# Bojian-Wei/Non-IID-Distributed-Learning-with-Optimal-Mixture-Weights

Measured on AMD Instinct MI355X. Metric: client-rounds/sec (whole node), higher is better.
Workload: dtype f32; 1 GPU; config 2: fedavg, 100 clients x 512 rows, RFF D=2048, C=10, E=2, B=32, 10000 test rows, round=1880, parallel clients; algo=fedavg, clients_total=100, clients_per_gpu=100, rows_per_client=512, D=2048, C=10, epochs=2, batch=32, test_rows=10000, parallelism=clients1

## Files before the change

non-iid-distributed-learning-with-optimal-mixture-weights_amd/_lib.py:

```python
import ctypes as C
import os

import torch

from . import LIB_PATH

_c_f32p = C.POINTER(C.c_float)
_SIGS = {
    'fs_abi_version': (C.c_int, []),
    'fs_last_error': (C.c_char_p, []),
    'fs_tuning_size': (C.c_int64, []),
    'fs_set_tuning': (C.c_int, [C.c_void_p]),
    'fs_set_thread_tuning': (C.c_int, [C.c_void_p]),
    'fs_get_tuning': (C.c_int, [C.c_void_p]),
    'fs_get_process_tuning': (C.c_int, [C.c_void_p]),
    'fs_get_thread_tuning': (C.c_int, [C.c_void_p]),
    'fs_randperm_batch': (C.c_int, [C.c_void_p, C.c_void_p, C.c_void_p, C.c_int64, C.c_void_p, C.c_int]),
    'fs_libsvm_scan': (C.c_int, [C.c_char_p, C.c_void_p, C.c_void_p, C.c_void_p]),
    'fs_libsvm_read': (C.c_int, [C.c_char_p, C.c_int64, C.c_int64, C.c_int, C.c_void_p, C.c_void_p, C.c_int]),
    'fs_randperm_device': (C.c_int, [C.c_void_p, C.c_void_p, C.c_void_p, C.c_int64, C.c_int64, C.c_void_p,
                                     C.c_void_p, C.c_void_p]),
    'fs_local_train_plan': (C.c_int, [C.c_int, C.c_int, C.c_int, C.c_int, C.c_int64, C.c_int64, C.c_int,
                                      C.c_int, C.c_void_p, C.c_void_p]),
    'fs_local_train': (C.c_int, [C.c_void_p, C.c_int64, C.c_void_p, C.c_void_p, C.c_void_p, C.c_void_p,
# ... 49 lines not shown
    'fs_plan_shuffle': (C.c_int, [C.c_void_p, C.c_void_p, C.c_int]),
    'fs_plan_round': (C.c_int, [C.c_void_p, C.c_int, C.c_float, C.c_int, C.c_void_p, C.c_void_p]),
    'fs_plan_eval_flush': (C.c_int, [C.c_void_p, C.c_void_p]),
    'fs_local_train_last_kernel': (C.c_int, []),
    'fs_plan_set_shuffle_chunk': (C.c_int, [C.c_void_p, C.c_int]),
    'fs_plan_shuffle_flush': (C.c_int, [C.c_void_p]),
    'fs_plan_eval_blocks': (C.c_int, [C.c_void_p]),
    'fs_timer_create': (C.c_int, [C.c_void_p]),
    'fs_timer_record': (C.c_int, [C.c_void_p, C.c_void_p]),
    'fs_timer_elapsed_ms': (C.c_int, [C.c_void_p, C.c_void_p, C.c_void_p]),
    'fs_timer_destroy': (C.c_int, [C.c_void_p]),
}

EXPORTS = tuple(_SIGS)
ABI_VERSION = 20

PHASE_TRAIN, PHASE_AGGREGATE, PHASE_EVAL, PHASE_EVAL_DEFER = 1, 2, 4, 8
G_PAIR = 256
G_TEAMS = 512
LT_KERNELS = {1: 'single', 2: 'split', 3: 'dbuf', 4: 'pair', 5: 'pipe', 6: 'teams', 7: 'mb'}
G_PIPE = 1024
ERR_BLOCK = 256
SOLVER_NAMES = {0: 'none', 1: 'reg', 2: 'mc', 3: 'staged', 4: 'global', 5: 'reg2', 6: 'wave', 8: 'quad', 9: 'qmc', 10: 'bin'}
SOLVERS = {v: k for k, v in SOLVER_NAMES.items() if k}


class Tuning(C.Structure):
    _fields_ = [('mix_solver', C.c_int), ('mix_prefetch', C.c_int), ('mix_prefetch_lead', C.c_int),
                ('mix_exact_softmax', C.c_int), ('no_eval_fuse', C.c_int), ('spin_limit', C.c_uint),
                ('inject_timeout', C.c_int), ('train_form', C.c_int),
                ('split_early', C.c_int), ('mix_qmc_lane_clients', C.c_int),
                ('mix_quad_loaders', C.c_int), ('split_teams', C.c_int),
                ('mix_poll_delay', C.c_int), ('split_poll_delay', C.c_int), ('split_pipe', C.c_int),
                ('split_dbuf', C.c_int),
                ('split_mb', C.c_int)]


class PlanDesc(C.Structure):
    _fields_ = [
        ('d_phi', C.c_void_p), ('ld', C.c_int64), ('d_row_off', C.c_void_p), ('d_labels', C.c_void_p),
        ('d_order', C.c_void_p), ('h_n', C.c_void_p),
        ('N', C.c_int), ('C', C.c_int), ('B', C.c_int), ('E', C.c_int), ('G', C.c_int),
        ('d_ws', C.c_void_p), ('ws_bytes', C.c_int64),
        ('chained', C.c_int), ('prox', C.c_int), ('reg', C.c_int), ('mu', C.c_float), ('lam', C.c_float),
        ('d_W_g', C.c_void_p), ('d_W_out', C.c_void_p), ('d_loss_hist', C.c_void_p),
        ('d_p', C.c_void_p), ('d_agg_ws', C.c_void_p), ('agg_ws_floats', C.c_int64), ('agg_chunks', C.c_int),
        ('d_phi_t', C.c_void_p), ('d_labels_t', C.c_void_p), ('n_t', C.c_int), ('d_eval_ws', C.c_void_p),
        ('d_eval_hist', C.c_void_p), ('shuffle_device', C.c_int), ('host_threads', C.c_int),
        ('shuffle_after_train', C.c_int),
        ('loss', C.c_int), ('d_y', C.c_void_p), ('d_y_t', C.c_void_p),
    ]

_lib = None


class FedsimError(RuntimeError):
    pass


def lib():
    global _lib
    if _lib is None:
        path = os.environ.get('FEDSIM_LIB') or LIB_PATH
        if not os.path.exists(path):
            raise FedsimError(
                'libfedsim.so not found at %s -- build it with `python -c "import __graft_entry__ as g; g.build()"` '
                'or `make -C <pkg>/csrc`; there is no CPU fallback' % path)
        h = C.CDLL(path, mode=C.RTLD_GLOBAL)
        for name, (res, args) in _SIGS.items():
            f = getattr(h, name)
            f.restype = res
            f.argtypes = args
        if h.fs_abi_version() != ABI_VERSION:
            raise FedsimError('libfedsim.so ABI %d != %d' % (h.fs_abi_version(), ABI_VERSION))
        if h.fs_tuning_size() != C.sizeof(Tuning):
            raise FedsimError('fs_tuning layout mismatch (%d != %d bytes)' % (h.fs_tuning_size(), C.sizeof(Tuning)))
        if h.fs_plan_desc_size() != C.sizeof(PlanDesc):
            raise FedsimError('fs_plan_desc layout mismatch (%d != %d bytes)' % (h.fs_plan_desc_size(),
                                                                                  C.sizeof(PlanDesc)))
        _lib = h
    return _lib


def get_tuning():
    t = Tuning()
    check(lib().fs_get_tuning(C.byref(t)), 'fs_get_tuning')
    return {k: getattr(t, k) for k, _ in Tuning._fields_}


def last_mix_layout():
    k, nk = C.c_int(0), C.c_int(0)
    check(lib().fs_mix_solve_last_layout(C.byref(k), C.byref(nk)), 'fs_mix_solve_last_layout')
    return k.value, nk.value


class MixPlan(C.Structure):
    _fields_ = [('solver', C.c_int), ('workgroups', C.c_int), ('lane_clients', C.c_int), ('helpers', C.c_int),
                ('lead', C.c_int), ('poll_delay', C.c_int), ('ws_bytes', C.c_int64)]


def mix_plan(N, C_, n_val, epochs, Bv, blocks=1):
    out = MixPlan()
    check(lib().fs_mix_solve_plan(int(N), int(C_), int(n_val), int(epochs), int(Bv), int(blocks), C.byref(out)),
          'fs_mix_solve_plan')
    return {k: getattr(out, k) for k, _ in MixPlan._fields_}


def get_process_tuning():
    t = Tuning()
    check(lib().fs_get_process_tuning(C.byref(t)), 'fs_get_process_tuning')
    return {k: getattr(t, k) for k, _ in Tuning._fields_}


def get_thread_tuning():
    t = Tuning()
    has = lib().fs_get_thread_tuning(C.byref(t))
    if has < 0:
        check(has, 'fs_get_thread_tuning')
    return {k: getattr(t, k) for k, _ in Tuning._fields_} if has else None


def _merged(base, fields):
    cur = dict(base)
    for k, v in fields.items():
        if k not in cur:
            raise KeyError('fs_tuning has no field %r' % k)
        if k == 'mix_solver' and isinstance(v, str):
            v = 0 if v == 'auto' else SOLVERS[v]
        cur[k] = int(v)
    return cur


def set_tuning(**fields):
    prev = get_process_tuning()
    check(lib().fs_set_tuning(C.byref(Tuning(**_merged(prev, fields)))), 'fs_set_tuning')
    return prev


def set_thread_tuning(fields=None):
    if fields is None:
        check(lib().fs_set_thread_tuning(None), 'fs_set_thread_tuning')
        return
    cur = _merged({k: 0 for k, _ in Tuning._fields_}, fields)
    check(lib().fs_set_thread_tuning(C.byref(Tuning(**cur))), 'fs_set_thread_tuning')


class tuning:

    def __init__(self, **fields):
        self.fields = fields

    def __enter__(self):
        own = get_thread_tuning()
        self.thread_prev = own
        if own is not None:
            set_thread_tuning(_merged(own, self.fields))
        else:
            self.prev = set_tuning(**self.fields)
        return self

    def __exit__(self, *exc):
        if self.thread_prev is not None:
            set_thread_tuning(self.thread_prev)
        else:
            check(lib().fs_set_tuning(C.byref(Tuning(**self.prev))), 'fs_set_tuning')
        return False
# ... 85 lines not shown
```

non-iid-distributed-learning-with-optimal-mixture-weights_amd/csrc/randperm.hip:

```cpp
#include "common.h"

namespace fs {

constexpr int MT_N = 624, MT_M = 397;
constexpr int RP_THREADS = 64;

__device__ __forceinline__ uint32_t mt_mix(uint32_t a, uint32_t b, uint32_t c) {
  const uint32_t y = (a & 0x80000000u) | (b & 0x7fffffffu);
  return c ^ (y >> 1) ^ ((y & 1u) ? 0x9908b0dfu : 0u);
}

__device__ __forceinline__ uint32_t mt_temper(uint32_t y) {
  y ^= y >> 11;
  y ^= (y << 7) & 0x9d2c5680u;
  y ^= (y << 15) & 0xefc60000u;
  y ^= y >> 18;
  return y;
}

__device__ void mt_twist(uint32_t* mt) {
  const int lane = threadIdx.x;
  uint32_t v[4];
#pragma unroll
  for (int k = 0; k < 4; ++k) {
    const int i = lane + 64 * k;
    if (i < MT_N - MT_M) v[k] = mt_mix(mt[i], mt[i + 1], mt[i + MT_M]);
  }
  __syncthreads();
#pragma unroll
  for (int k = 0; k < 4; ++k) {
    const int i = lane + 64 * k;
    if (i < MT_N - MT_M) mt[i] = v[k];
  }
  __syncthreads();
#pragma unroll
  for (int k = 0; k < 4; ++k) {
    const int i = (MT_N - MT_M) + lane + 64 * k;
    if (i < 2 * (MT_N - MT_M)) v[k] = mt_mix(mt[i], mt[i + 1], mt[i + MT_M - MT_N]);
  }
  __syncthreads();
#pragma unroll
  for (int k = 0; k < 4; ++k) {
    const int i = (MT_N - MT_M) + lane + 64 * k;
    if (i < 2 * (MT_N - MT_M)) mt[i] = v[k];
  }
  __syncthreads();
#pragma unroll
  for (int k = 0; k < 3; ++k) {
    const int i = 2 * (MT_N - MT_M) + lane + 64 * k;
    if (i < MT_N - 1) v[k] = mt_mix(mt[i], mt[i + 1], mt[i + MT_M - MT_N]);
  }
  __syncthreads();
#pragma unroll
  for (int k = 0; k < 3; ++k) {
    const int i = 2 * (MT_N - MT_M) + lane + 64 * k;
    if (i < MT_N - 1) mt[i] = v[k];
  }
  __syncthreads();
  if (lane == 0) mt[MT_N - 1] = mt_mix(mt[MT_N - 1], mt[0], mt[MT_M - 1]);
  __syncthreads();
}

__device__ __forceinline__ void rp_contract_broken(int32_t* dst, int n, int lane, int stride, uint32_t* err) {
  for (int i = lane; i < n; i += stride) dst[i] = i;
  if (err && lane == 0) __hip_atomic_store(err, 1u, __ATOMIC_RELAXED, __HIP_MEMORY_SCOPE_AGENT);
}

template <bool IN_LDS>
__global__ __launch_bounds__(RP_THREADS) void randperm_kernel(const int64_t* __restrict__ seeds,
                                                             const int64_t* __restrict__ ns,
                                                             const int64_t* __restrict__ offs,
                                                             int32_t* __restrict__ out, int64_t max_n,
                                                             uint32_t* err) {
  extern __shared__ __attribute__((aligned(16))) uint32_t smem_rp[];
  uint32_t* mt = smem_rp;
  uint32_t* rnd = mt + MT_N;
  const int lane = threadIdx.x;
  const int pass = blockIdx.x;
  const int64_t n64 = ns[pass];
  int32_t* dst = out + offs[pass];
  if (n64 > max_n) {
    rp_contract_broken(dst, (int)n64, lane, RP_THREADS, err);
    return;
  }
  const int n = (int)n64;
  int32_t* perm = IN_LDS ? reinterpret_cast<int32_t*>(rnd + MT_N) : dst;
  for (int i = lane; i < n; i += RP_THREADS) perm[i] = i;
  if (lane == 0) {
    uint32_t x = (uint32_t)(uint64_t)seeds[pass];
    mt[0] = x;
    for (int i = 1; i < MT_N; ++i) {
      x = 1812433253u * (x ^ (x >> 30)) + (uint32_t)i;
      mt[i] = x;
    }
  }
  __syncthreads();
  for (int i0 = 0; i0 < n - 1; i0 += MT_N) {
    mt_twist(mt);
    for (int k = lane; k < MT_N; k += RP_THREADS) rnd[k] = mt_temper(mt[k]);
    __syncthreads();
    if (lane == 0) {
      const int i1 = min(n - 1, i0 + MT_N);
      for (int i = i0; i < i1; ++i) {
        const uint32_t z = rnd[i - i0] % (uint32_t)(n - i);
        const int32_t a = perm[i];
        perm[i] = perm[i + z];
        perm[i + z] = a;
      }
    }
    __syncthreads();
  }
  if (IN_LDS)
    for (int i = lane; i < n; i += RP_THREADS) dst[i] = perm[i];
}

constexpr int RL_MAXN = 64;

__global__ __launch_bounds__(64) void randperm_lanes_kernel(const int64_t* __restrict__ seeds,
                                                           const int64_t* __restrict__ ns,
                                                           const int64_t* __restrict__ offs, int64_t npasses,
                                                           int32_t* __restrict__ out, int max_n, uint32_t* err) {
  __shared__ int32_t perm_s[64][RL_MAXN + 1];
  const int lane = threadIdx.x;
  const int64_t pass = (int64_t)blockIdx.x * 64 + lane;
  const bool live = pass < npasses;
  const int n_req = live ? (int)ns[pass] : 0;
  const int n = n_req <= max_n ? n_req : 0;
  if (n_req > max_n && err) __hip_atomic_store(err, 1u, __ATOMIC_RELAXED, __HIP_MEMORY_SCOPE_AGENT);
  int32_t* perm = perm_s[lane];
  uint32_t lo[RL_MAXN], hi[RL_MAXN - 1];
  {
    uint32_t x = live ? (uint32_t)(uint64_t)seeds[pass] : 0u;
    lo[0] = x;
#pragma unroll
    for (int i = 1; i <= MT_M + RL_MAXN - 2; ++i) {
      x = 1812433253u * (x ^ (x >> 30)) + (uint32_t)i;
      if (i < RL_MAXN) lo[i] = x;
      if (i >= MT_M) hi[i - MT_M] = x;
    }
  }
#pragma unroll
  for (int i = 0; i < RL_MAXN; ++i)
    if (i < n) perm[i] = i;
#pragma unroll
  for (int i = 0; i < RL_MAXN - 1; ++i) {
    if (i < n - 1) {
      const uint32_t r = mt_temper(mt_mix(lo[i], lo[i + 1], hi[i]));
      const int z = (int)(r % (uint32_t)(n - i));
      const int32_t a = perm[i];
      perm[i] = perm[i + z];
      perm[i + z] = a;
    }
  }
  if (live) {
    int32_t* dst = out + offs[pass];
    for (int i = 0; i < n; ++i) dst[i] = perm[i];
    for (int i = n; i < n_req; ++i) dst[i] = i;
  }
}

}

using namespace fs;

extern "C" int fs_randperm_device(const int64_t* d_seeds, const int64_t* d_n, const int64_t* d_off, int64_t npasses,
                                  int64_t max_n, int32_t* d_out, uint32_t* d_err, void* stream) {
  FS_REQUIRE(npasses >= 0 && max_n >= 0 && max_n < ((int64_t)1 << 31), "bad sizes");
  if (npasses == 0) return FS_OK;
  FS_REQUIRE(d_seeds && d_n && d_off && d_out, "null pointer");
  hipStream_t st = reinterpret_cast<hipStream_t>(stream);
  if (max_n <= RL_MAXN) {
    hipLaunchKernelGGL(randperm_lanes_kernel, dim3((unsigned)((npasses + 63) / 64)), dim3(64), 0, st, d_seeds, d_n,
                       d_off, npasses, d_out, (int)max_n, d_err);
    FS_LAUNCH_CHECK();
    return FS_OK;
  }
  const size_t lds_small = sizeof(uint32_t) * 2 * MT_N;
  const size_t lds_full = lds_small + sizeof(int32_t) * (size_t)max_n;
  if (lds_full <= 160 * 1024) {
    if (lds_full > 64 * 1024) {
      hipError_t e = hipFuncSetAttribute(reinterpret_cast<const void*>(&randperm_kernel<true>),
                                         hipFuncAttributeMaxDynamicSharedMemorySize, (int)lds_full);
      if (e != hipSuccess) return fail(FS_EHIP, std::string("fs_randperm_device: ") + hipGetErrorString(e));
    }
    hipLaunchKernelGGL(randperm_kernel<true>, dim3((unsigned)npasses), dim3(RP_THREADS), lds_full, st, d_seeds, d_n,
                       d_off, d_out, max_n, d_err);
  } else {
    hipLaunchKernelGGL(randperm_kernel<false>, dim3((unsigned)npasses), dim3(RP_THREADS), lds_small, st, d_seeds, d_n,
                       d_off, d_out, max_n, d_err);
  }
  FS_LAUNCH_CHECK();
  return FS_OK;
}
```

non-iid-distributed-learning-with-optimal-mixture-weights_amd/csrc/round.hip:

```cpp
#include <hip/hip_runtime.h>

#include <algorithm>
#include <atomic>
#include <condition_variable>
#include <cstring>
#include <functional>
#include <mutex>
#include <deque>
#include <thread>
#include <vector>

#include <chrono>
#include <cstdio>

#include "common.h"
#include "finalize.h"
#include "mse_rows.h"
#include "mt_replay.h"

namespace fs {

class Pool {
 public:
  explicit Pool(int nthreads) {
    for (int t = 1; t < nthreads; ++t) th_.emplace_back([this] { loop(); });
  }
  ~Pool() {
    {
      std::lock_guard<std::mutex> lk(m_);
      stop_ = true;
      ++gen_;
    }
    cv_.notify_all();
    for (auto& t : th_) t.join();
  }
  void run(int64_t n, const std::function<void(int64_t)>& fn) {
    if (th_.empty() || n <= 1) {
      for (int64_t i = 0; i < n; ++i) fn(i);
      return;
    }
    {
      std::lock_guard<std::mutex> lk(m_);
      fn_ = &fn;
      n_ = n;
      next_.store(0);
      busy_ = (int)th_.size();
      ++gen_;
    }
    cv_.notify_all();
    work();
    std::unique_lock<std::mutex> lk(m_);
    done_.wait(lk, [this] { return busy_ == 0; });
    fn_ = nullptr;
  }

 private:
  void work() {
    for (;;) {
      const int64_t i = next_.fetch_add(1);
      if (i >= n_) return;
      (*fn_)(i);
    }
  }
  void loop() {
    uint64_t seen = 0;
    for (;;) {
      {
        std::unique_lock<std::mutex> lk(m_);
        cv_.wait(lk, [&] { return gen_ != seen; });
        seen = gen_;
        if (stop_) return;
      }
      work();
      std::lock_guard<std::mutex> lk(m_);
      if (--busy_ == 0) done_.notify_all();
    }
  }
  std::vector<std::thread> th_;
  std::mutex m_;
  std::condition_variable cv_, done_;
  const std::function<void(int64_t)>* fn_ = nullptr;
  int64_t n_ = 0;
  std::atomic<int64_t> next_{0};
  int busy_ = 0;
  uint64_t gen_ = 0;
  bool stop_ = false;
};

}

struct fs_plan {
  fs_plan_desc d;
  std::vector<int64_t> n, off;
  int64_t perm_len = 0;
  int32_t* h_perm[2] = {nullptr, nullptr};
  int32_t* d_perm[2] = {nullptr, nullptr};
  static constexpr int SEED_SLOTS = 4;
  int64_t* h_seed[SEED_SLOTS] = {};
  int64_t* d_seed[SEED_SLOTS] = {};
  int64_t* h_seed_dev[SEED_SLOTS] = {};
  hipEvent_t seed_read[SEED_SLOTS] = {};
  bool seed_pending[SEED_SLOTS] = {};
  bool seed_copy = false;
  int64_t* d_pass = nullptr;
  int64_t max_n = 0;
  int64_t max_client_steps = 0;
  int fuse_E = 0;
  int eval_pending = -1;
  int fin_pending = -1;
  hipStream_t copy = nullptr;
  hipEvent_t uploaded[2] = {nullptr, nullptr};
  hipEvent_t consumed[2] = {nullptr, nullptr};
  bool up_pending[2] = {false, false};
  bool cons_recorded[2] = {false, false};
  int slot_round[2] = {-1, -1};
  int chunk = 1;
  int64_t* d_pass_chunk = nullptr;
  int slot_chunk[2] = {-1, -1};
  int slot_nrounds[2] = {0, 0};
  int slot_waited[2] = {-1, -1};
  int fill_chunk = -1, fill_rounds = 0;
  int job_status = FS_OK;
  std::string job_error;
  fs::Pool* pool = nullptr;
  std::thread coord;
  std::mutex m;
  std::condition_variable cv, done;
  std::deque<std::pair<int, std::vector<int64_t>>> jobs;
  bool stop = false;
};

using namespace fs;

static int hip_fail(const char* what, hipError_t e) {
  return fail(FS_EHIP, std::string(what) + ": " + hipGetErrorString(e));
}

#define FS_HIP(call, what)                          \
  do {                                              \
    hipError_t e_ = (call);                         \
    if (e_ != hipSuccess) return hip_fail(what, e_); \
  } while (0)

extern "C" int64_t fs_plan_desc_size(void) { return (int64_t)sizeof(fs_plan_desc); }

static int run_shuffle_job(fs_plan* p, const int64_t* h_seeds, int t);

static void coordinator(fs_plan* p) {
  for (;;) {
    std::pair<int, std::vector<int64_t>> job;
    {
      std::unique_lock<std::mutex> lk(p->m);
      p->cv.wait(lk, [p] { return p->stop || !p->jobs.empty(); });
      if (p->jobs.empty()) return;
      job = std::move(p->jobs.front());
    }
    const int rc = run_shuffle_job(p, job.second.data(), job.first);
    std::lock_guard<std::mutex> lk(p->m);
    p->jobs.pop_front();
    if (rc != FS_OK && p->job_status == FS_OK) {
      p->job_status = rc;
      p->job_error = fs_last_error();
    }
    p->done.notify_all();
  }
}

extern "C" int fs_plan_destroy(fs_plan* p) {
  if (!p) return FS_OK;
  if (p->coord.joinable()) {
    {
      std::lock_guard<std::mutex> lk(p->m);
      p->stop = true;
    }
    p->cv.notify_all();
    p->coord.join();
  }
  if (p->copy) (void)hipStreamSynchronize(p->copy);
  for (int s = 0; s < 2; ++s) {
    if (p->h_perm[s]) (void)hipHostFree(p->h_perm[s]);
    if (p->d_perm[s]) (void)hipFree(p->d_perm[s]);
    if (p->uploaded[s]) (void)hipEventDestroy(p->uploaded[s]);
    if (p->consumed[s]) (void)hipEventDestroy(p->consumed[s]);
  }
  for (int s = 0; s < fs_plan::SEED_SLOTS; ++s) {
    if (p->h_seed[s]) (void)hipHostFree(p->h_seed[s]);
    if (p->d_seed[s]) (void)hipFree(p->d_seed[s]);
    if (p->seed_read[s]) (void)hipEventDestroy(p->seed_read[s]);
  }
  if (p->d_pass) (void)hipFree(p->d_pass);
  if (p->d_pass_chunk) (void)hipFree(p->d_pass_chunk);
  if (p->copy) (void)hipStreamDestroy(p->copy);
  delete p->pool;
  delete p;
  return FS_OK;
}

extern "C" int fs_plan_create(const fs_plan_desc* desc, fs_plan** out) {
  FS_REQUIRE(desc && out, "null pointer");
  const fs_plan_desc& d = *desc;
  FS_REQUIRE(d.N >= 1 && d.E >= 0 && d.C >= 1 && d.ld >= 64 && d.ld % 64 == 0, "bad sizes");
  FS_REQUIRE(d.loss == 0 || d.loss == 1, "loss must be 0 (cross-entropy) or 1 (MSE)");
  FS_REQUIRE(d.h_n && d.d_phi && d.d_row_off && (d.loss ? (const void*)d.d_y : (const void*)d.d_labels) && d.d_W_g &&
                 d.d_W_out && d.d_loss_hist,
             "null pointer");
  FS_REQUIRE(d.loss == 0 || (d.C == 1 && d.G == 1), "the MSE plan needs C == 1 and G == 1");
  *out = nullptr;
  fs_plan* p = new fs_plan();
  p->d = d;
  int64_t rows = 0;
  for (int j = 0; j < d.N; ++j) {
    if (d.h_n[j] < 0) {
      delete p;
      return fail(FS_EINVAL, "fs_plan_create: negative client size");
    }
    for (int e = 0; e < d.E; ++e) {
      p->n.push_back(d.h_n[j]);
      p->off.push_back((int64_t)d.E * rows + (int64_t)e * d.h_n[j]);
    }
    rows += d.h_n[j];
  }
  p->perm_len = std::max<int64_t>(1, (int64_t)d.E * rows);
  const int64_t P = (int64_t)p->n.size();
  for (int64_t v : p->n) p->max_n = std::max(p->max_n, v);
  {
    int64_t mx = 0;
    for (int j = 0; j < d.N; ++j) mx = std::max(mx, d.h_n[j]);
    p->max_client_steps = std::max<int64_t>(1, (int64_t)d.E * ((mx + d.B - 1) / std::max(1, d.B)));
  }
  if (d.loss == 0 && d.d_phi_t && d.n_t > 0 && d.d_labels_t && d.d_eval_ws && d.C <= 16 && d.G > 1 && !d.chained) {
    if (!fs::tuning().no_eval_fuse) {
      const int idle = fs::split_idle_cus(d.N, d.C, d.B, d.ld, d.G, 0);
      p->fuse_E = (int)std::min<int64_t>(idle, (d.n_t + 15) / 16);
    }
  }
  hipError_t e = hipSuccess;
  for (int s = 0; s < 2 && e == hipSuccess; ++s) {
    if (!d.shuffle_device) {
      e = hipHostMalloc(reinterpret_cast<void**>(&p->h_perm[s]), sizeof(int32_t) * p->perm_len, hipHostMallocDefault);
    }
    if (e == hipSuccess) e = hipMalloc(reinterpret_cast<void**>(&p->d_perm[s]), sizeof(int32_t) * p->perm_len);
    const unsigned evf = hipEventDisableTiming | (unsigned)hipEventDisableSystemFence;
    if (e == hipSuccess) e = hipEventCreateWithFlags(&p->uploaded[s], evf);
    if (e == hipSuccess) e = hipEventCreateWithFlags(&p->consumed[s], evf);
  }
  if (d.shuffle_device) {
    p->seed_copy = false;
    for (int k = 0; k < fs_plan::SEED_SLOTS && e == hipSuccess; ++k) {
      e = hipHostMalloc(reinterpret_cast<void**>(&p->h_seed[k]), sizeof(int64_t) * std::max<int64_t>(1, P),
                        p->seed_copy ? hipHostMallocDefault : (hipHostMallocMapped | hipHostMallocCoherent));
      if (e == hipSuccess && !p->seed_copy)
        e = hipHostGetDevicePointer(reinterpret_cast<void**>(&p->h_seed_dev[k]), p->h_seed[k], 0);
      if (e == hipSuccess) e = hipMalloc(reinterpret_cast<void**>(&p->d_seed[k]), sizeof(int64_t) * std::max<int64_t>(1, P));
      if (e == hipSuccess) e = hipEventCreateWithFlags(&p->seed_read[k], hipEventDisableTiming | hipEventDisableSystemFence);
    }
  }
  if (e == hipSuccess) e = hipStreamCreateWithFlags(&p->copy, hipStreamNonBlocking);
  if (e == hipSuccess && d.shuffle_device && P > 0) {
    std::vector<int64_t> h(2 * P);
    std::copy(p->n.begin(), p->n.end(), h.begin());
    std::copy(p->off.begin(), p->off.end(), h.begin() + P);
    e = hipMalloc(reinterpret_cast<void**>(&p->d_pass), sizeof(int64_t) * 2 * P);
    if (e == hipSuccess) e = hipMemcpy(p->d_pass, h.data(), sizeof(int64_t) * 2 * P, hipMemcpyHostToDevice);
  }
  if (e != hipSuccess) {
    fs_plan_destroy(p);
    return hip_fail("fs_plan_create", e);
  }
  if (!d.shuffle_device) {
    const int nthreads =
        d.host_threads > 0 ? d.host_threads : (int)std::min(16u, std::max(1u, std::thread::hardware_concurrency()));
    p->pool = new Pool(nthreads);
    int dev = 0;
    (void)hipGetDevice(&dev);
    p->coord = std::thread([p, dev] {
      (void)hipSetDevice(dev);
      coordinator(p);
    });
  }
  *out = p;
  return FS_OK;
}

static int device_shuffle(fs_plan* p, const int64_t* h_seeds, int t) {
  const int s = t & 1;
  const int64_t P = (int64_t)p->n.size();
  const int k = t % fs_plan::SEED_SLOTS;
  if (p->seed_pending[k]) FS_HIP(hipEventSynchronize(p->seed_read[k]), "fs_plan_shuffle");
  std::memcpy(p->h_seed[k], h_seeds, sizeof(int64_t) * P);
  if (p->cons_recorded[s]) FS_HIP(hipStreamWaitEvent(p->copy, p->consumed[s], 0), "fs_plan_shuffle");
  if (p->d.shuffle_after_train && p->cons_recorded[s ^ 1])
    FS_HIP(hipStreamWaitEvent(p->copy, p->consumed[s ^ 1], 0), "fs_plan_shuffle");
  if (p->seed_copy)
    FS_HIP(hipMemcpyAsync(p->d_seed[k], p->h_seed[k], sizeof(int64_t) * P, hipMemcpyHostToDevice, p->copy),
           "fs_plan_shuffle");
  const int64_t* seeds = p->seed_copy ? p->d_seed[k] : p->h_seed_dev[k];
  const int rc = fs_randperm_device(seeds, p->d_pass, p->d_pass + P, P, p->max_n, p->d_perm[s], nullptr, p->copy);
  if (rc != FS_OK) return rc;
  FS_HIP(hipEventRecord(p->seed_read[k], p->copy), "fs_plan_shuffle");
  p->seed_pending[k] = true;
  FS_HIP(hipEventRecord(p->uploaded[s], p->copy), "fs_plan_shuffle");
  p->up_pending[s] = true;
  p->slot_round[s] = t;
  return FS_OK;
}

extern "C" int fs_plan_set_shuffle_chunk(fs_plan* p, int rounds) {
  FS_REQUIRE(p && rounds >= 1 && rounds <= 64, "bad arguments");
  FS_REQUIRE(p->d.shuffle_device, "fs_plan_set_shuffle_chunk: device replay only");
  FS_REQUIRE(!p->seed_pending[0] && p->slot_round[0] < 0 && p->slot_round[1] < 0 && p->slot_chunk[0] < 0 &&
                 p->fill_chunk < 0,
             "fs_plan_set_shuffle_chunk: set before the first shuffle");
  if (rounds == p->chunk) return FS_OK;
  const int64_t P = (int64_t)p->n.size();
  const int64_t KP = std::max<int64_t>(1, (int64_t)rounds * P);
  for (int s = 0; s < 2; ++s) {
    FS_HIP(hipFree(p->d_perm[s]), "fs_plan_set_shuffle_chunk");
    p->d_perm[s] = nullptr;
    FS_HIP(hipMalloc(reinterpret_cast<void**>(&p->d_perm[s]), sizeof(int32_t) * p->perm_len * rounds),
           "fs_plan_set_shuffle_chunk");
  }
  for (int k = 0; k < fs_plan::SEED_SLOTS; ++k) {
    FS_HIP(hipHostFree(p->h_seed[k]), "fs_plan_set_shuffle_chunk");
    FS_HIP(hipFree(p->d_seed[k]), "fs_plan_set_shuffle_chunk");
    p->h_seed[k] = nullptr;
    p->d_seed[k] = nullptr;
    FS_HIP(hipHostMalloc(reinterpret_cast<void**>(&p->h_seed[k]), sizeof(int64_t) * KP,
                         p->seed_copy ? hipHostMallocDefault : (hipHostMallocMapped | hipHostMallocCoherent)),
           "fs_plan_set_shuffle_chunk");
    if (!p->seed_copy)
      FS_HIP(hipHostGetDevicePointer(reinterpret_cast<void**>(&p->h_seed_dev[k]), p->h_seed[k], 0),
             "fs_plan_set_shuffle_chunk");
    FS_HIP(hipMalloc(reinterpret_cast<void**>(&p->d_seed[k]), sizeof(int64_t) * KP), "fs_plan_set_shuffle_chunk");
  }
  if (p->d_pass_chunk) FS_HIP(hipFree(p->d_pass_chunk), "fs_plan_set_shuffle_chunk");
  p->d_pass_chunk = nullptr;
  if (P > 0) {
    std::vector<int64_t> h(2 * KP);
    for (int r = 0; r < rounds; ++r)
      for (int64_t i = 0; i < P; ++i) {
        h[r * P + i] = p->n[i];
        h[KP + r * P + i] = p->off[i] + (int64_t)r * p->perm_len;
      }
    FS_HIP(hipMalloc(reinterpret_cast<void**>(&p->d_pass_chunk), sizeof(int64_t) * 2 * KP),
           "fs_plan_set_shuffle_chunk");
    FS_HIP(hipMemcpy(p->d_pass_chunk, h.data(), sizeof(int64_t) * 2 * KP, hipMemcpyHostToDevice),
           "fs_plan_set_shuffle_chunk");
  }
  p->chunk = rounds;
  return FS_OK;
}

static int launch_chunk(fs_plan* p) {
  const int c = p->fill_chunk, nr = p->fill_rounds, K = p->chunk;
  const int s = c & 1, k = c % fs_plan::SEED_SLOTS;
  const int64_t P = (int64_t)p->n.size(), KP = std::max<int64_t>(1, (int64_t)K * P);
  if (p->cons_recorded[s]) FS_HIP(hipStreamWaitEvent(p->copy, p->consumed[s], 0), "fs_plan_shuffle");
  if (P > 0) {
    if (p->seed_copy)
      FS_HIP(hipMemcpyAsync(p->d_seed[k], p->h_seed[k], sizeof(int64_t) * nr * P, hipMemcpyHostToDevice, p->copy),
             "fs_plan_shuffle");
    const int64_t* seeds = p->seed_copy ? p->d_seed[k] : p->h_seed_dev[k];
    const int rc = fs_randperm_device(seeds, p->d_pass_chunk, p->d_pass_chunk + KP, nr * P, p->max_n, p->d_perm[s],
                                      nullptr, p->copy);
    if (rc != FS_OK) return rc;
  }
  FS_HIP(hipEventRecord(p->seed_read[k], p->copy), "fs_plan_shuffle");
  p->seed_pending[k] = true;
  FS_HIP(hipEventRecord(p->uploaded[s], p->copy), "fs_plan_shuffle");
  p->up_pending[s] = true;
  p->slot_chunk[s] = c;
  p->slot_nrounds[s] = nr;
  p->fill_chunk = -1;
  p->fill_rounds = 0;
  return FS_OK;
}

static int chunk_shuffle(fs_plan* p, const int64_t* h_seeds, int t) {
  const int K = p->chunk, c = t / K, r = t % K;
  const int64_t P = (int64_t)p->n.size();
  FS_REQUIRE(r == (p->fill_chunk == c ? p->fill_rounds : 0) && (r > 0 || p->fill_chunk < 0),
             "rounds must be prepared in order");
  if (r == 0) {
    const int k = c % fs_plan::SEED_SLOTS;
    if (p->seed_pending[k]) FS_HIP(hipEventSynchronize(p->seed_read[k]), "fs_plan_shuffle");
    p->fill_chunk = c;
    p->fill_rounds = 0;
  }
  std::memcpy(p->h_seed[c % fs_plan::SEED_SLOTS] + (int64_t)r * P, h_seeds, sizeof(int64_t) * P);
  ++p->fill_rounds;
  return r == K - 1 ? launch_chunk(p) : FS_OK;
}

extern "C" int fs_timer_create(void** ev) {
  FS_REQUIRE(ev, "null pointer");
  hipEvent_t e = nullptr;
  FS_HIP(hipEventCreateWithFlags(&e, (unsigned)hipEventDisableSystemFence), "fs_timer_create");
  *ev = e;
  return FS_OK;
}
extern "C" int fs_timer_record(void* ev, void* stream) {
  FS_REQUIRE(ev, "null pointer");
  FS_HIP(hipEventRecord(reinterpret_cast<hipEvent_t>(ev), reinterpret_cast<hipStream_t>(stream)), "fs_timer_record");
  return FS_OK;
}
extern "C" int fs_timer_elapsed_ms(void* start, void* end, float* ms) {
  FS_REQUIRE(start && end && ms, "null pointer");
  FS_HIP(hipEventSynchronize(reinterpret_cast<hipEvent_t>(end)), "fs_timer_elapsed_ms");
  FS_HIP(hipEventElapsedTime(ms, reinterpret_cast<hipEvent_t>(start), reinterpret_cast<hipEvent_t>(end)),
         "fs_timer_elapsed_ms");
  return FS_OK;
}
extern "C" int fs_timer_destroy(void* ev) {
  if (ev) FS_HIP(hipEventDestroy(reinterpret_cast<hipEvent_t>(ev)), "fs_timer_destroy");
  return FS_OK;
}

extern "C" int fs_plan_eval_blocks(const fs_plan* p) {
  FS_REQUIRE(p, "bad arguments");
  return p->fuse_E;
}

extern "C" int fs_plan_shuffle_flush(fs_plan* p) {
  FS_REQUIRE(p, "bad arguments");
  return (p->chunk > 1 && p->fill_chunk >= 0) ? launch_chunk(p) : FS_OK;
}

extern "C" int fs_plan_shuffle(fs_plan* p, const int64_t* h_seeds, int t) {
  FS_REQUIRE(p && (h_seeds || p->n.empty()) && t >= 0, "bad arguments");
  if (p->d.shuffle_device) {
    if (p->chunk > 1) return chunk_shuffle(p, h_seeds, t);
    if (p->n.empty()) {
      p->slot_round[t & 1] = t;
      return FS_OK;
    }
    return device_shuffle(p, h_seeds, t);
  }
  {
    std::lock_guard<std::mutex> lk(p->m);
    if (p->job_status != FS_OK) return fail(p->job_status, p->job_error);
    p->jobs.emplace_back(t, std::vector<int64_t>(h_seeds, h_seeds + p->n.size()));
  }
  p->cv.notify_all();
  return FS_OK;
}

static int run_shuffle_job(fs_plan* p, const int64_t* h_seeds, int t) {
// ... 136 lines not shown
```

non-iid-distributed-learning-with-optimal-mixture-weights_amd/engine.py:

```python
import numpy as np
import torch

from . import _lib


def pad_ld(D):
    return max(64, (int(D) + 63) // 64 * 64)


def _to_device_f32(xs, device):
    if len(xs) == 1:
        return xs[0].to(device=device, dtype=torch.float32, non_blocking=True)
    if all(x.is_cuda for x in xs):
        return torch.cat([x.to(device=device, dtype=torch.float32) for x in xs], 0)
    return torch.cat([x.detach().to('cpu', torch.float32) for x in xs], 0).to(device, non_blocking=True)


class Features:

    def __init__(self, X_list, y_list, D, device, ld=None, float_targets=False):
        self.device = device
        self.D = int(D)
        self.ld = ld or pad_ld(D)
        self.ns = np.array([int(len(y)) for y in y_list], dtype=np.int64)
        self.row_off = np.concatenate([[0], np.cumsum(self.ns)]).astype(np.int64)
        rows = int(self.row_off[-1])
        self.rows = rows
        for X in X_list:
            if X.dim() != 2 or X.shape[1] != self.D:
                raise ValueError('feature matrix must be [n, D=%d], got %s' % (self.D, tuple(X.shape)))
        self.phi = torch.zeros(max(rows, 1), self.ld, device=device, dtype=torch.float32)
        tdt = torch.float32 if float_targets else torch.int32
        if rows:
            self.phi[:rows, :self.D].copy_(_to_device_f32([torch.as_tensor(x) for x in X_list], device))
            y = torch.cat([torch.as_tensor(v).reshape(-1).to('cpu', torch.float32 if float_targets else torch.int64)
                           for v in y_list])
            tgt = y.to(tdt).to(device)
        else:
            tgt = torch.zeros(1, dtype=tdt, device=device)
        self.labels = None if float_targets else tgt
        self.y = tgt if float_targets else None
        self.targets = tgt
        self.row_off_dev = torch.from_numpy(self.row_off).to(device)


class Shuffler:

    def __init__(self, ns, offs, size, device, max_n=None):
        self.P = int(len(ns))
        self.max_n = int(max_n) if max_n is not None else (int(np.max(ns)) if self.P else 0)
        self.err = torch.zeros(_lib.ERR_BLOCK // 4, dtype=torch.int32, device=device)
        self.n_dev = torch.as_tensor(np.asarray(ns, dtype=np.int64)).to(device)
        self.off_dev = torch.as_tensor(np.asarray(offs, dtype=np.int64)).to(device)
        self.bufs = [torch.empty(max(1, int(size)), dtype=torch.int32, device=device) for _ in range(2)]
        self.seed_dev = [torch.empty(max(1, self.P), dtype=torch.int64, device=device) for _ in range(2)]
        self.seed_host = [torch.empty(max(1, self.P), dtype=torch.int64, pin_memory=True) for _ in range(2)]
        self.host_free = [None, None]
        self.ready = [None, None]
        self.consumed = [None, None]

    def prepare(self, seeds, slot, stream=None):
        stream = stream or torch.cuda.current_stream()
        seeds = np.asarray(seeds, dtype=np.int64)
        assert seeds.shape == (self.P,)
        if self.host_free[slot] is not None:
            self.host_free[slot].synchronize()
        self.seed_host[slot].numpy()[:] = seeds
        if self.consumed[slot] is not None:
            stream.wait_event(self.consumed[slot])
        with torch.cuda.stream(stream):
            self.seed_dev[slot].copy_(self.seed_host[slot], non_blocking=True)
            ev = torch.cuda.Event()
            ev.record(stream)
            self.host_free[slot] = ev
            if self.P:
                _lib.check(_lib.lib().fs_randperm_device(_lib.ptr(self.seed_dev[slot]), _lib.ptr(self.n_dev),
                                                         _lib.ptr(self.off_dev), self.P, self.max_n,
                                                         _lib.ptr(self.bufs[slot]), _lib.ptr(self.err),
                                                         _lib.stream_ptr(stream)),
                           'fs_randperm_device')
            ready = torch.cuda.Event()
            ready.record(stream)
        self.ready[slot] = ready

    def acquire(self, slot):
        torch.cuda.current_stream().wait_event(self.ready[slot])
        return self.bufs[slot]

    def release(self, slot):
        ev = torch.cuda.Event()
        ev.record()
        self.consumed[slot] = ev

    def run(self, seeds, slot=0):
        self.prepare(seeds, slot)
        return self.acquire(slot)

    def check_errors(self):
        err = int(self.err[0].item())
        if err:
            self.err.zero_()
            raise _lib.FedsimError('fs_randperm_device: a pass is longer than max_n = %d; it was written as the '
                                   'identity permutation (code %d)' % (self.max_n, err))


def _check_ws_error(ws, what):
    if ws is None:
        return
    blk = ws[ws.numel() - _lib.ERR_BLOCK:]
    err = int(blk[:4].view(torch.int32).item())
    if err:
        blk.zero_()
        raise _lib.FedsimError('%s: a cross-workgroup hand-off timed out (code %d); results are invalid' % (what, err))


class LocalTrainer:

    def __init__(self, feats, C, B, E, split=None, chained=False, rows=None, prox=False, loss='ce'):
        if loss not in ('ce', 'mse'):
            raise ValueError("loss must be 'ce' or 'mse'")
        self.task = loss
        if loss == 'mse' and (int(C) != 1 or feats.y is None):
            raise ValueError("loss='mse' needs C == 1 and Features(float_targets=True)")
        if loss == 'ce' and feats.labels is None:
            raise ValueError("loss='ce' needs integer labels")
        self.f = feats
        self.C, self.B, self.E = int(C), int(B), int(E)
        dev = feats.device
        N = len(feats.ns)
        self.N = N
        self.chained = bool(chained)
        self.W_out = torch.zeros(max(N, int(rows or 0)), self.C, feats.ld, device=dev, dtype=torch.float32)
        self.loss = torch.zeros(N, device=dev, dtype=torch.float64)
        ns = feats.ns
        self.pass_n = np.repeat(ns, self.E)
        self.pass_off = (np.repeat(self.E * feats.row_off[:-1], self.E)
                         + np.tile(np.arange(self.E), N) * np.repeat(ns, self.E)).astype(np.int64)
        self._shuffler = None
        steps = self.E * ((ns + self.B - 1) // self.B)
        order = np.argsort(-steps, kind='stable').astype(np.int32)
        self.order = torch.from_numpy(order).to(dev)
        if loss == 'mse':
            if split not in (None, 1):
                raise _lib.FedsimError('fs_local_train_mse has no split form (one workgroup per client)')
            self.G, self.pair, self.teams, self.pipe, self.width, self.ws = 1, False, False, False, 1, None
            return
        import ctypes
        g, wsb = ctypes.c_int(0 if split is None else int(split)), ctypes.c_int64(0)
        max_en = int(self.E * ns.max()) if N else 0
        _lib.check(_lib.lib().fs_local_train_plan(N, self.C, self.B, self.E, feats.ld, max_en, int(self.chained),
                                                  int(bool(prox)), ctypes.byref(g), ctypes.byref(wsb)),
                   'fs_local_train_plan')
        if split is not None and int(split) != g.value:
            raise _lib.FedsimError('fs_local_train_plan: G=%d is not available for this shape (planner: %d)'
                                   % (int(split), g.value))
        self.G = int(g.value)
        self.pair = bool(self.G & _lib.G_PAIR)
        self.teams = bool(self.G & _lib.G_TEAMS)
# ... 392 lines not shown
```

Before: 363,500 client-rounds/s.

## Cap device randperm grid to idle CUs with multi-wave persistent blocks

Adds a capped randperm path that launches a limited, XCD-aware number of persistent blocks. Each block packs several waves, and each wave handles its own shuffle pass in its own LDS region, syncing with wave barriers instead of workgroup barriers. The block count comes from the idle CUs left over by the training split, so the shuffle can overlap with local training on the copy stream instead of competing for the whole GPU. The trade-off is fewer blocks doing more passes each. The Python side reaches the new entry point through a mangled C++ symbol, which is fragile.

```diff
diff --git a/non-iid-distributed-learning-with-optimal-mixture-weights_amd/_lib.py b/non-iid-distributed-learning-with-optimal-mixture-weights_amd/_lib.py
--- a/non-iid-distributed-learning-with-optimal-mixture-weights_amd/_lib.py
+++ b/non-iid-distributed-learning-with-optimal-mixture-weights_amd/_lib.py
@@ -155,6 +155,20 @@
     return _lib
 
 
+_randperm_capped = None
+
+
+def randperm_device_capped():
+    global _randperm_capped
+    if _randperm_capped is None:
+        f = getattr(lib(), '_ZN2fs15randperm_deviceEPKlS1_S1_llPiPjiPv')
+        f.restype = C.c_int
+        f.argtypes = [C.c_void_p, C.c_void_p, C.c_void_p, C.c_int64, C.c_int64, C.c_void_p, C.c_void_p, C.c_int,
+                      C.c_void_p]
+        _randperm_capped = f
+    return _randperm_capped
+
+
 def get_tuning():
     t = Tuning()
     check(lib().fs_get_tuning(C.byref(t)), 'fs_get_tuning')
diff --git a/non-iid-distributed-learning-with-optimal-mixture-weights_amd/csrc/randperm.hip b/non-iid-distributed-learning-with-optimal-mixture-weights_amd/csrc/randperm.hip
--- a/non-iid-distributed-learning-with-optimal-mixture-weights_amd/csrc/randperm.hip
+++ b/non-iid-distributed-learning-with-optimal-mixture-weights_amd/csrc/randperm.hip
@@ -1,8 +1,9 @@
 #include "common.h"
+#include "randperm_geom.h"
 
 namespace fs {
 
-constexpr int MT_N = 624, MT_M = 397;
+constexpr int MT_N = RP_MT_N, MT_M = 397;
 constexpr int RP_THREADS = 64;
 
 __device__ __forceinline__ uint32_t mt_mix(uint32_t a, uint32_t b, uint32_t c) {
@@ -18,52 +19,105 @@
   return y;
 }
 
-__device__ void mt_twist(uint32_t* mt) {
-  const int lane = threadIdx.x;
+template <bool WG>
+__device__ __forceinline__ void rp_sync() {
+  if (WG) {
+    __syncthreads();
+  } else {
+    asm volatile("s_waitcnt lgkmcnt(0)" ::: "memory");
+    __builtin_amdgcn_wave_barrier();
+    asm volatile("" ::: "memory");
+  }
+}
+
+template <bool WG>
+__device__ __forceinline__ void mt_twist(uint32_t* mt, int lane) {
   uint32_t v[4];
 #pragma unroll
   for (int k = 0; k < 4; ++k) {
     const int i = lane + 64 * k;
     if (i < MT_N - MT_M) v[k] = mt_mix(mt[i], mt[i + 1], mt[i + MT_M]);
   }
-  __syncthreads();
+  rp_sync<WG>();
 #pragma unroll
   for (int k = 0; k < 4; ++k) {
     const int i = lane + 64 * k;
     if (i < MT_N - MT_M) mt[i] = v[k];
   }
-  __syncthreads();
+  rp_sync<WG>();
 #pragma unroll
   for (int k = 0; k < 4; ++k) {
     const int i = (MT_N - MT_M) + lane + 64 * k;
     if (i < 2 * (MT_N - MT_M)) v[k] = mt_mix(mt[i], mt[i + 1], mt[i + MT_M - MT_N]);
   }
-  __syncthreads();
+  rp_sync<WG>();
 #pragma unroll
   for (int k = 0; k < 4; ++k) {
     const int i = (MT_N - MT_M) + lane + 64 * k;
     if (i < 2 * (MT_N - MT_M)) mt[i] = v[k];
   }
-  __syncthreads();
+  rp_sync<WG>();
 #pragma unroll
   for (int k = 0; k < 3; ++k) {
     const int i = 2 * (MT_N - MT_M) + lane + 64 * k;
     if (i < MT_N - 1) v[k] = mt_mix(mt[i], mt[i + 1], mt[i + MT_M - MT_N]);
   }
-  __syncthreads();
+  rp_sync<WG>();
 #pragma unroll
   for (int k = 0; k < 3; ++k) {
     const int i = 2 * (MT_N - MT_M) + lane + 64 * k;
     if (i < MT_N - 1) mt[i] = v[k];
   }
-  __syncthreads();
+  rp_sync<WG>();
   if (lane == 0) mt[MT_N - 1] = mt_mix(mt[MT_N - 1], mt[0], mt[MT_M - 1]);
-  __syncthreads();
+  rp_sync<WG>();
 }
 
 __device__ __forceinline__ void rp_contract_broken(int32_t* dst, int n, int lane, int stride, uint32_t* err) {
   for (int i = lane; i < n; i += stride) dst[i] = i;
   if (err && lane == 0) __hip_atomic_store(err, 1u, __ATOMIC_RELAXED, __HIP_MEMORY_SCOPE_AGENT);
+}
+
+template <bool IN_LDS, bool WG>
+__device__ __forceinline__ void rp_pass(uint32_t* mt, uint32_t* rnd, int32_t* perm_lds,
+                                        const int64_t* __restrict__ seeds, const int64_t* __restrict__ ns,
+                                        const int64_t* __restrict__ offs, int32_t* __restrict__ out, int64_t max_n,
+                                        uint32_t* err, int64_t pass, int lane) {
+  const int64_t n64 = ns[pass];
+  int32_t* dst = out + offs[pass];
+  if (n64 > max_n) {
+    rp_contract_broken(dst, (int)n64, lane, RP_THREADS, err);
+    return;
+  }
+  const int n = (int)n64;
+  int32_t* perm = IN_LDS ? perm_lds : dst;
+  for (int i = lane; i < n; i += RP_THREADS) perm[i] = i;
+  if (lane == 0) {
+    uint32_t x = (uint32_t)(uint64_t)seeds[pass];
+    mt[0] = x;
+    for (int i = 1; i < MT_N; ++i) {
+      x = 1812433253u * (x ^ (x >> 30)) + (uint32_t)i;
+      mt[i] = x;
+    }
+  }
+  rp_sync<WG>();
+  for (int i0 = 0; i0 < n - 1; i0 += MT_N) {
+    mt_twist<WG>(mt, lane);
+    for (int k = lane; k < MT_N; k += RP_THREADS) rnd[k] = mt_temper(mt[k]);
+    rp_sync<WG>();
+    if (lane == 0) {
+      const int i1 = min(n - 1, i0 + MT_N);
+      for (int i = i0; i < i1; ++i) {
+        const uint32_t z = rnd[i - i0] % (uint32_t)(n - i);
+        const int32_t a = perm[i];
+        perm[i] = perm[i + z];
+        perm[i + z] = a;
+      }
+    }
+    rp_sync<WG>();
+  }
+  if (IN_LDS)
+    for (int i = lane; i < n; i += RP_THREADS) dst[i] = perm[i];
 }
 
 template <bool IN_LDS>
@@ -75,54 +129,33 @@
   extern __shared__ __attribute__((aligned(16))) uint32_t smem_rp[];
   uint32_t* mt = smem_rp;
   uint32_t* rnd = mt + MT_N;
-  const int lane = threadIdx.x;
-  const int pass = blockIdx.x;
-  const int64_t n64 = ns[pass];
-  int32_t* dst = out + offs[pass];
-  if (n64 > max_n) {
-    rp_contract_broken(dst, (int)n64, lane, RP_THREADS, err);
-    return;
-  }
-  const int n = (int)n64;
-  int32_t* perm = IN_LDS ? reinterpret_cast<int32_t*>(rnd + MT_N) : dst;
-  for (int i = lane; i < n; i += RP_THREADS) perm[i] = i;
-  if (lane == 0) {
-    uint32_t x = (uint32_t)(uint64_t)seeds[pass];
-    mt[0] = x;
-    for (int i = 1; i < MT_N; ++i) {
-      x = 1812433253u * (x ^ (x >> 30)) + (uint32_t)i;
-      mt[i] = x;
-    }
-  }
-  __syncthreads();
-  for (int i0 = 0; i0 < n - 1; i0 += MT_N) {
-    mt_twist(mt);
-    for (int k = lane; k < MT_N; k += RP_THREADS) rnd[k] = mt_temper(mt[k]);
-    __syncthreads();
-    if (lane == 0) {
-      const int i1 = min(n - 1, i0 + MT_N);
-      for (int i = i0; i < i1; ++i) {
-        const uint32_t z = rnd[i - i0] % (uint32_t)(n - i);
-        const int32_t a = perm[i];
-        perm[i] = perm[i + z];
-        perm[i + z] = a;
-      }
-    }
-    __syncthreads();
-  }
-  if (IN_LDS)
-    for (int i = lane; i < n; i += RP_THREADS) dst[i] = perm[i];
+  rp_pass<IN_LDS, true>(mt, rnd, reinterpret_cast<int32_t*>(rnd + MT_N), seeds, ns, offs, out, max_n, err,
+                        blockIdx.x, threadIdx.x);
+}
+
+__global__ __launch_bounds__(RP_THREADS * RP_MAX_WAVES) void randperm_capped_kernel(
+    const int64_t* __restrict__ seeds, const int64_t* __restrict__ ns, const int64_t* __restrict__ offs,
+    int64_t npasses, int32_t* __restrict__ out, int64_t max_n, uint32_t* err, int region) {
+  extern __shared__ __attribute__((aligned(16))) uint32_t smem_rp[];
+  const int lane = threadIdx.x & (RP_THREADS - 1);
+  const int wave = __builtin_amdgcn_readfirstlane(threadIdx.x / RP_THREADS);
+  const int waves = blockDim.x / RP_THREADS;
+  uint32_t* mt = smem_rp + (size_t)wave * region;
+  uint32_t* rnd = mt + MT_N;
+  const int64_t total = (int64_t)gridDim.x * waves;
+  for (int64_t pass = (int64_t)blockIdx.x * waves + wave; pass < npasses; pass += total) {
+    rp_pass<true, false>(mt, rnd, reinterpret_cast<int32_t*>(rnd + MT_N), seeds, ns, offs, out, max_n, err, pass, lane);
+    rp_sync<false>();
+  }
 }
 
 constexpr int RL_MAXN = 64;
 
-__global__ __launch_bounds__(64) void randperm_lanes_kernel(const int64_t* __restrict__ seeds,
-                                                           const int64_t* __restrict__ ns,
-                                                           const int64_t* __restrict__ offs, int64_t npasses,
-                                                           int32_t* __restrict__ out, int max_n, uint32_t* err) {
-  __shared__ int32_t perm_s[64][RL_MAXN + 1];
-  const int lane = threadIdx.x;
-  const int64_t pass = (int64_t)blockIdx.x * 64 + lane;
+__device__ __forceinline__ void rl_block(int32_t (*perm_s)[RL_MAXN + 1], const int64_t* __restrict__ seeds,
+                                         const int64_t* __restrict__ ns, const int64_t* __restrict__ offs,
+                                         int64_t npasses, int32_t* __restrict__ out, int max_n, uint32_t* err,
+                                         int64_t blk, int lane) {
+  const int64_t pass = blk * 64 + lane;
   const bool live = pass < npasses;
   const int n_req = live ? (int)ns[pass] : 0;
   const int n = n_req <= max_n ? n_req : 0;
@@ -159,19 +192,53 @@
   }
 }
 
-}
-
-using namespace fs;
-
-extern "C" int fs_randperm_device(const int64_t* d_seeds, const int64_t* d_n, const int64_t* d_off, int64_t npasses,
-                                  int64_t max_n, int32_t* d_out, uint32_t* d_err, void* stream) {
-  FS_REQUIRE(npasses >= 0 && max_n >= 0 && max_n < ((int64_t)1 << 31), "bad sizes");
+__global__ __launch_bounds__(64) void randperm_lanes_kernel(const int64_t* __restrict__ seeds,
+                                                           const int64_t* __restrict__ ns,
+                                                           const int64_t* __restrict__ offs, int64_t npasses,
+                                                           int32_t* __restrict__ out, int max_n, uint32_t* err) {
+  __shared__ int32_t perm_s[64][RL_MAXN + 1];
+  rl_block(perm_s, seeds, ns, offs, npasses, out, max_n, err, blockIdx.x, threadIdx.x);
+}
+
+__global__ __launch_bounds__(64) void randperm_lanes_capped_kernel(const int64_t* __restrict__ seeds,
+                                                                  const int64_t* __restrict__ ns,
+                                                                  const int64_t* __restrict__ offs, int64_t npasses,
+                                                                  int32_t* __restrict__ out, int max_n,
+                                                                  uint32_t* err) {
+  __shared__ int32_t perm_s[64][RL_MAXN + 1];
+  for (int64_t blk = blockIdx.x; blk * 64 < npasses; blk += gridDim.x)
+    rl_block(perm_s, seeds, ns, offs, npasses, out, max_n, err, blk, threadIdx.x);
+}
+
+}
+
+namespace fs {
+
+int randperm_device(const int64_t* d_seeds, const int64_t* d_n, const int64_t* d_off, int64_t npasses, int64_t max_n,
+                    int32_t* d_out, uint32_t* d_err, int max_blocks, void* stream) {
+  FS_REQUIRE(npasses >= 0 && max_n >= 0 && max_n < ((int64_t)1 << 31) && max_blocks >= 0, "bad sizes");
   if (npasses == 0) return FS_OK;
   FS_REQUIRE(d_seeds && d_n && d_off && d_out, "null pointer");
   hipStream_t st = reinterpret_cast<hipStream_t>(stream);
   if (max_n <= RL_MAXN) {
-    hipLaunchKernelGGL(randperm_lanes_kernel, dim3((unsigned)((npasses + 63) / 64)), dim3(64), 0, st, d_seeds, d_n,
-                       d_off, npasses, d_out, (int)max_n, d_err);
+    if (max_blocks > 0)
+      hipLaunchKernelGGL(randperm_lanes_capped_kernel, dim3((unsigned)rp_capped_lanes_geom(npasses, max_blocks).blocks),
+                         dim3(64), 0, st, d_seeds, d_n, d_off, npasses, d_out, (int)max_n, d_err);
+    else
+      hipLaunchKernelGGL(randperm_lanes_kernel, dim3((unsigned)((npasses + 63) / 64)), dim3(64), 0, st, d_seeds, d_n,
+                         d_off, npasses, d_out, (int)max_n, d_err);
+    FS_LAUNCH_CHECK();
+    return FS_OK;
+  }
+  if (max_blocks > 0 && rp_in_lds(max_n)) {
+    const RpGeom g = rp_capped_geom(npasses, max_n, max_blocks);
+    if (g.lds > 64 * 1024) {
+      hipError_t e = hipFuncSetAttribute(reinterpret_cast<const void*>(&randperm_capped_kernel),
+                                         hipFuncAttributeMaxDynamicSharedMemorySize, (int)g.lds);
+      if (e != hipSuccess) return fail(FS_EHIP, std::string("fs_randperm_device: ") + hipGetErrorString(e));
+    }
+    hipLaunchKernelGGL(randperm_capped_kernel, dim3((unsigned)g.blocks), dim3(RP_THREADS * g.waves), (size_t)g.lds, st,
+                       d_seeds, d_n, d_off, npasses, d_out, max_n, d_err, (int)rp_region_words(max_n, true));
     FS_LAUNCH_CHECK();
     return FS_OK;
   }
@@ -192,3 +259,12 @@
   FS_LAUNCH_CHECK();
   return FS_OK;
 }
+
+}
+
+using namespace fs;
+
+extern "C" int fs_randperm_device(const int64_t* d_seeds, const int64_t* d_n, const int64_t* d_off, int64_t npasses,
+                                  int64_t max_n, int32_t* d_out, uint32_t* d_err, void* stream) {
+  return fs::randperm_device(d_seeds, d_n, d_off, npasses, max_n, d_out, d_err, 0, stream);
+}
diff --git a/non-iid-distributed-learning-with-optimal-mixture-weights_amd/csrc/randperm_geom.h b/non-iid-distributed-learning-with-optimal-mixture-weights_amd/csrc/randperm_geom.h
--- /dev/null
+++ b/non-iid-distributed-learning-with-optimal-mixture-weights_amd/csrc/randperm_geom.h
@@ -0,0 +1,60 @@
+#pragma once
+
+#include <algorithm>
+#include <cstdint>
+
+namespace fs {
+
+constexpr int RP_MT_N = 624;
+constexpr int RP_MAX_WAVES = 16;
+constexpr int64_t RP_LDS_BYTES = 160 * 1024;
+constexpr int RP_LANE_PASSES = 64;
+constexpr int RP_XCDS = 8;
+
+inline int64_t rp_region_words(int64_t max_n, bool in_lds) {
+  return (2 * (int64_t)RP_MT_N + (in_lds ? max_n : 0) + 3) / 4 * 4;
+}
+
+inline bool rp_in_lds(int64_t max_n) { return 4 * (2 * (int64_t)RP_MT_N + max_n) <= RP_LDS_BYTES; }
+
+inline int rp_waves(int64_t max_n) {
+  if (max_n <= RP_LANE_PASSES) return 1;
+  const int64_t region = 4 * rp_region_words(max_n, rp_in_lds(max_n));
+  return (int)std::max<int64_t>(1, std::min<int64_t>(RP_MAX_WAVES, RP_LDS_BYTES / region));
+}
+
+inline int rp_cap_blocks(int idle, int64_t npasses, int64_t max_n, int rounds) {
+  if (!rp_in_lds(max_n)) return 0;
+  const int per_xcd = idle / RP_XCDS / 2;
+  const int64_t unit = max_n <= RP_LANE_PASSES ? RP_LANE_PASSES : 1;
+  const int64_t turns = (npasses + unit - 1) / unit;
+  const int waves = rp_waves(max_n);
+  for (int take = 1; take <= per_xcd; ++take) {
+    const int64_t w = (int64_t)RP_XCDS * take * waves;
+    if ((turns + w - 1) / w <= std::max(1, rounds)) return RP_XCDS * take;
+  }
+  return 0;
+}
+
+struct RpGeom {
+  int blocks;
+  int waves;
+  int64_t lds;
+};
+
+inline RpGeom rp_capped_geom(int64_t npasses, int64_t max_n, int max_blocks) {
+  const int64_t region = 4 * rp_region_words(max_n, rp_in_lds(max_n));
+  const int waves = rp_waves(max_n);
+  const int64_t need = (npasses + waves - 1) / waves;
+  return {(int)std::max<int64_t>(1, std::min<int64_t>(max_blocks, need)), waves, region * waves};
+}
+
+inline RpGeom rp_capped_lanes_geom(int64_t npasses, int max_blocks) {
+  const int64_t need = (npasses + RP_LANE_PASSES - 1) / RP_LANE_PASSES;
+  return {(int)std::max<int64_t>(1, std::min<int64_t>(max_blocks, need)), 1, 0};
+}
+
+int randperm_device(const int64_t* d_seeds, const int64_t* d_n, const int64_t* d_off, int64_t npasses, int64_t max_n,
+                    int32_t* d_out, uint32_t* d_err, int max_blocks, void* stream);
+
+}
diff --git a/non-iid-distributed-learning-with-optimal-mixture-weights_amd/csrc/round.hip b/non-iid-distributed-learning-with-optimal-mixture-weights_amd/csrc/round.hip
--- a/non-iid-distributed-learning-with-optimal-mixture-weights_amd/csrc/round.hip
+++ b/non-iid-distributed-learning-with-optimal-mixture-weights_amd/csrc/round.hip
@@ -17,6 +17,11 @@
 #include "finalize.h"
 #include "mse_rows.h"
 #include "mt_replay.h"
+#include "randperm_geom.h"
+
+#ifndef RP_CAPPED
+#define RP_CAPPED 1
+#endif
 
 namespace fs {
 
@@ -106,6 +111,7 @@
   int64_t max_n = 0;
   int64_t max_client_steps = 0;
   int fuse_E = 0;
+  int rp_idle = 0;
   int eval_pending = -1;
   int fin_pending = -1;
   hipStream_t copy = nullptr;
@@ -234,6 +240,8 @@
       p->fuse_E = (int)std::min<int64_t>(idle, (d.n_t + 15) / 16);
     }
   }
+  if (RP_CAPPED && d.shuffle_device && d.loss == 0 && d.G > 1 && !d.chained && !d.shuffle_after_train)
+    p->rp_idle = fs::split_idle_cus(d.N, d.C, d.B, d.ld, d.G, 0);
   hipError_t e = hipSuccess;
   for (int s = 0; s < 2 && e == hipSuccess; ++s) {
     if (!d.shuffle_device) {
@@ -280,6 +288,10 @@
   }
   *out = p;
   return FS_OK;
+}
+
+static int plan_rp_cap(const fs_plan* p, int64_t npasses, int rounds) {
+  return fs::rp_cap_blocks(p->rp_idle, npasses, p->max_n, rounds);
 }
 
 static int device_shuffle(fs_plan* p, const int64_t* h_seeds, int t) {
@@ -295,7 +307,8 @@
     FS_HIP(hipMemcpyAsync(p->d_seed[k], p->h_seed[k], sizeof(int64_t) * P, hipMemcpyHostToDevice, p->copy),
            "fs_plan_shuffle");
   const int64_t* seeds = p->seed_copy ? p->d_seed[k] : p->h_seed_dev[k];
-  const int rc = fs_randperm_device(seeds, p->d_pass, p->d_pass + P, P, p->max_n, p->d_perm[s], nullptr, p->copy);
+  const int rc = fs::randperm_device(seeds, p->d_pass, p->d_pass + P, P, p->max_n, p->d_perm[s], nullptr,
+                                     plan_rp_cap(p, P, 1), p->copy);
   if (rc != FS_OK) return rc;
   FS_HIP(hipEventRecord(p->seed_read[k], p->copy), "fs_plan_shuffle");
   p->seed_pending[k] = true;
@@ -361,8 +374,8 @@
       FS_HIP(hipMemcpyAsync(p->d_seed[k], p->h_seed[k], sizeof(int64_t) * nr * P, hipMemcpyHostToDevice, p->copy),
              "fs_plan_shuffle");
     const int64_t* seeds = p->seed_copy ? p->d_seed[k] : p->h_seed_dev[k];
-    const int rc = fs_randperm_device(seeds, p->d_pass_chunk, p->d_pass_chunk + KP, nr * P, p->max_n, p->d_perm[s],
-                                      nullptr, p->copy);
+    const int rc = fs::randperm_device(seeds, p->d_pass_chunk, p->d_pass_chunk + KP, nr * P, p->max_n, p->d_perm[s],
+                                       nullptr, plan_rp_cap(p, nr * P, nr), p->copy);
     if (rc != FS_OK) return rc;
   }
   FS_HIP(hipEventRecord(p->seed_read[k], p->copy), "fs_plan_shuffle");
diff --git a/non-iid-distributed-learning-with-optimal-mixture-weights_amd/engine.py b/non-iid-distributed-learning-with-optimal-mixture-weights_amd/engine.py
--- a/non-iid-distributed-learning-with-optimal-mixture-weights_amd/engine.py
+++ b/non-iid-distributed-learning-with-optimal-mixture-weights_amd/engine.py
@@ -46,8 +46,9 @@
 
 class Shuffler:
 
-    def __init__(self, ns, offs, size, device, max_n=None):
+    def __init__(self, ns, offs, size, device, max_n=None, max_blocks=0):
         self.P = int(len(ns))
+        self.max_blocks = int(max_blocks)
         self.max_n = int(max_n) if max_n is not None else (int(np.max(ns)) if self.P else 0)
         self.err = torch.zeros(_lib.ERR_BLOCK // 4, dtype=torch.int32, device=device)
         self.n_dev = torch.as_tensor(np.asarray(ns, dtype=np.int64)).to(device)
@@ -73,7 +74,13 @@
             ev = torch.cuda.Event()
             ev.record(stream)
             self.host_free[slot] = ev
-            if self.P:
+            if self.P and self.max_blocks > 0:
+                _lib.check(_lib.randperm_device_capped()(_lib.ptr(self.seed_dev[slot]), _lib.ptr(self.n_dev),
+                                                         _lib.ptr(self.off_dev), self.P, self.max_n,
+                                                         _lib.ptr(self.bufs[slot]), _lib.ptr(self.err),
+                                                         self.max_blocks, _lib.stream_ptr(stream)),
+                           'fs::randperm_device')
+            elif self.P:
                 _lib.check(_lib.lib().fs_randperm_device(_lib.ptr(self.seed_dev[slot]), _lib.ptr(self.n_dev),
                                                          _lib.ptr(self.off_dev), self.P, self.max_n,
                                                          _lib.ptr(self.bufs[slot]), _lib.ptr(self.err),
```

New measurement: 376,900 client-rounds/s, median of 6. +3.7%, better.
